# Sinica-SLAM/speechbrain

Hardware: AMD Instinct MI355X
Metric: audio-sec/sec Fbank→Conformer fwd (16kHz, B=32×15s) at 1/2/4/8 GPU (higher is better)
Workload: dtype bf16; 1 GPU; Fbank(80)→ConvFrontEnd(64,32)→Conformer 12L d=256 H=4 ffn=1024 k=31 encode, B=32×15s per GPU; global_batch=32, seq_len=376, parallelism=replicas1, hip_graph=True

## Files before the change

### speechbrain_amd/csrc/ffn.hip

```cpp
#include "mfma.h"

using namespace sbk;

namespace {

enum Act { ACT_NONE = 0, ACT_SWISH = 1, ACT_GLU = 2, ACT_LRELU = 3, ACT_GELU = 4 };

struct FfnArgs {
  const float* x;
  int M, H;
  const float *g0, *b0;
  float eps0;
  const bf16_t* img;
  const float* b1;
  int act;
  float slope;
  const float* b2;
  float alpha;
  const float *gp, *bp;
  float epsp;
  float* out;
  const float *gn, *bn;
  float epsn;
  void* u;
  int u_bf16;
  int np;
  bf16_t* yp;
  const float *g0b, *b0b;
  float eps0b;
  const float *b1b, *b2b;
  float alphab;
  float inv_n, npad;
  const bf16_t *sa, *simg;
  const float* sbias;
  int Kin, Tm;
  const float* rel_len;
  uint8_t* kpm_out;
};

__device__ __forceinline__ bf16x8 ld8(const bf16_t* p) { return *reinterpret_cast<const bf16x8*>(p); }

template <int V>
struct IntC {
  static constexpr int value = V;
};

constexpr int FFN_BM = 48;
#ifndef FFN_XCD_ORDER
#define FFN_XCD_ORDER 1
#endif
constexpr int FFN_PAD = 16;
constexpr int FFN_NW = 8, FFN_NT = FFN_NW * 64;
__device__ __forceinline__ constexpr int ffn_sw(int row) { return ((row >> 2) & 1) << 3; }
static_assert(FFN_NW % 8 == 0, "rows w + FFN_NW * i share bit 2 with w (their swizzle is ffn_sw(w))");
constexpr int FFN_RS = 12;

typedef float v2f __attribute__((ext_vector_type(2)));

#define FFN_MFMA(A, B, C) __builtin_amdgcn_mfma_f32_16x16x32_bf16((A), (B), (C), 0, 0, 0)

template <int ACT>
__device__ __forceinline__ float act_fn(float v, float slope) {
  if (ACT == ACT_SWISH) return v * __builtin_amdgcn_rcpf(1.0f + __expf(-v));
  if (ACT == ACT_LRELU) return v >= 0.f ? v : v * slope;
  if (ACT == ACT_GELU) return 0.5f * v * (1.0f + erff(v * 0.70710678118654752f));
  return v;
}

__device__ __forceinline__ f32x4 lds_f4(const float* p) {
  f32x4 v;
  const uint32_t la = (uint32_t)(uintptr_t)((const __attribute__((address_space(3))) float*)p);
  asm volatile("ds_read_b128 %0, %1" : "=v"(v) : "v"(la) : "memory");
  return v;
}

__device__ __forceinline__ uint32_t lds_addr(const void* p) {
  return (uint32_t)(uintptr_t)((const __attribute__((address_space(3))) char*)p);
}
__device__ __forceinline__ float lds_f1(const float* p) {
  float v;
  asm volatile("ds_read_b32 %0, %1" : "=v"(v) : "v"(lds_addr(p)) : "memory");
  return v;
}
__device__ __forceinline__ void lds_st1(float* p, float v) {
  asm volatile("ds_write_b32 %0, %1" ::"v"(lds_addr(p)), "v"(v) : "memory");
}
__device__ __forceinline__ void lds_st4(float* p, f32x4 v) {
  asm volatile("ds_write_b128 %0, %1" ::"v"(lds_addr(p)), "v"(v) : "memory");
}
__device__ __forceinline__ void lds_st2(void* p, uint2 v) {
  const unsigned long long u = (unsigned long long)v.x | ((unsigned long long)v.y << 32);
  asm volatile("ds_write_b64 %0, %1" ::"v"(lds_addr(p)), "v"(u) : "memory");
}
template <typename V>
__device__ __forceinline__ void tie(V& v) {
  asm volatile("s_waitcnt lgkmcnt(0)" : "+v"(v));
}
__device__ __forceinline__ void lds_barrier() {
  asm volatile("s_waitcnt lgkmcnt(0)" ::: "memory");
  __builtin_amdgcn_s_barrier();
}

__device__ __forceinline__ f32x4 gld4(const float* p) {
  f32x4 v;
  asm volatile("global_load_dwordx4 %0, %1, off" : "=v"(v) : "v"(p) : "memory");
  return v;
}
__device__ __forceinline__ void vtie(f32x4& v) { asm volatile("" : "+v"(v)); }

__device__ __forceinline__ void vm_wait(int n) {
  switch (n) {
    case 0: asm volatile("s_waitcnt vmcnt(0)" ::: "memory"); break;
    case 1: asm volatile("s_waitcnt vmcnt(1)" ::: "memory"); break;
    case 2: asm volatile("s_waitcnt vmcnt(2)" ::: "memory"); break;
    case 3: asm volatile("s_waitcnt vmcnt(3)" ::: "memory"); break;
    case 4: asm volatile("s_waitcnt vmcnt(4)" ::: "memory"); break;
    case 5: asm volatile("s_waitcnt vmcnt(5)" ::: "memory"); break;
    case 6: asm volatile("s_waitcnt vmcnt(6)" ::: "memory"); break;
    case 7: asm volatile("s_waitcnt vmcnt(7)" ::: "memory"); break;
    default: asm volatile("s_waitcnt vmcnt(8)" ::: "memory"); break;
  }
}

template <int D, int T2, int MT, int NW>
__device__ __forceinline__ void row_ln(float (&z)[T2][MT][4], float* red, const float* gam, const float* bet, float eps,
                                       int w, int g, int fr, float inv_n, float npad) {
  static_assert(NW == 8, "two b128 reads per row");
  float mean[MT], rstd[MT];
#pragma unroll
  for (int pass = 0; pass < 2; ++pass) {
    float part[MT];
#pragma unroll
    for (int mt = 0; mt < MT; ++mt) {
      float s = 0.f;
#pragma unroll
      for (int j = 0; j < T2; ++j)
#pragma unroll
        for (int e = 0; e < 4; ++e) {
          const float dv = pass ? z[j][mt][e] - mean[mt] : z[j][mt][e];
          s += pass ? dv * dv : dv;
        }
      part[mt] = col4_sum(s);
    }
    lds_barrier();
    if (g == 0) {
#pragma unroll
      for (int mt = 0; mt < MT; ++mt) lds_st1(red + (mt * 16 + fr) * FFN_RS + w, part[mt]);
    }
    lds_barrier();
    f32x4 rv[MT][2];
#pragma unroll
    for (int mt = 0; mt < MT; ++mt) {
      rv[mt][0] = lds_f4(red + (mt * 16 + fr) * FFN_RS);
      rv[mt][1] = lds_f4(red + (mt * 16 + fr) * FFN_RS + 4);
    }
#pragma unroll
    for (int mt = 0; mt < MT; ++mt) {
      tie(rv[mt][0]);
      tie(rv[mt][1]);
      const float t = (rv[mt][0][0] + rv[mt][0][1]) + (rv[mt][0][2] + rv[mt][0][3]) + (rv[mt][1][0] + rv[mt][1][1]) +
                      (rv[mt][1][2] + rv[mt][1][3]);
      if (pass)
        rstd[mt] = __builtin_amdgcn_rsqf((t - npad * mean[mt] * mean[mt]) * inv_n + eps);
      else
        mean[mt] = t * inv_n;
    }
  }
  f32x4 gv[T2], bv[T2];
#pragma unroll
  for (int j = 0; j < T2; ++j) {
    const int d = (w * T2 + j) * 16 + 4 * g;
    gv[j] = lds_f4(gam + d);
    bv[j] = lds_f4(bet + d);
  }
#pragma unroll
  for (int j = 0; j < T2; ++j) {
    tie(gv[j]);
    tie(bv[j]);
#pragma unroll
    for (int e = 0; e < 4; e += 2)
#pragma unroll
      for (int mt = 0; mt < MT; ++mt) {
        const v2f y = (v2f{z[j][mt][e], z[j][mt][e + 1]} - v2f{mean[mt], mean[mt]}) * v2f{rstd[mt], rstd[mt]} *
                          v2f{gv[j][e], gv[j][e + 1]} + v2f{bv[j][e], bv[j][e + 1]};
        z[j][mt][e] = y[0];
        z[j][mt][e + 1] = y[1];
      }
  }
}

__device__ __forceinline__ uint4 proj_pair(const f32x4& v0, const f32x4& v1) {
  const uint32_t a0 = pack_bf16x2(v0[0], v0[1]), a1 = pack_bf16x2(v0[2], v0[3]);
  const uint32_t b0 = pack_bf16x2(v1[0], v1[1]), b1 = pack_bf16x2(v1[2], v1[3]);
  const auto lo = __builtin_amdgcn_permlane16_swap(a0, b0, false, false);
  const auto hi = __builtin_amdgcn_permlane16_swap(a1, b1, false, false);
  return make_uint4(lo[0], hi[0], lo[1], hi[1]);
}

template <int K1, int KS, int MT, int XS, int BK>
__device__ __forceinline__ void load_frags(bf16x8 (&xa)[K1][KS][MT], const bf16_t* Xn, int fr, int fk) {
#pragma unroll
  for (int r = 0; r < K1; ++r)
#pragma unroll
    for (int ks = 0; ks < KS; ++ks)
#pragma unroll
      for (int mt = 0; mt < MT; ++mt)
        asm volatile("ds_read_b128 %0, %1"
                     : "=v"(xa[r][ks][mt])
                     : "v"(lds_addr(Xn + (mt * 16 + fr) * XS + r * BK + ks * 32 + fk))
                     : "memory");
#pragma unroll
  for (int r = 0; r < K1; ++r)
#pragma unroll
    for (int ks = 0; ks < KS; ++ks)
#pragma unroll
      for (int mt = 0; mt < MT; ++mt) tie(xa[r][ks][mt]);
}

SBK_PROBE_BUFFER(g_ffn_tl, 16, 256)
#define FFN_TL(i) SBK_PROBE(if (tl_rec >= 0 && lane == 0) g_ffn_tl[tl_rec][i] = __builtin_amdgcn_s_memtime();)

#include "convstage.h"

template <int D, int ACT, bool PROJ, bool CHAIN, bool CONV, bool SRC = false>
__device__ __forceinline__ void ffn_body(const FfnArgs& a, const ConvStageArgs* cs) {
  static_assert(!(CONV && SRC), "one kind of prologue");
  constexpr int BM = FFN_BM, HC = 256, NW = FFN_NW, NT = FFN_NT;
  constexpr int XS = D + FFN_PAD, HS = HC + FFN_PAD;
  constexpr int MT = BM / 16;
  constexpr int T = 256 / 16 / FFN_NW;
  constexpr int BK = 64;
  constexpr int K1 = D / BK, K2 = HC / BK, SPC = K1 + K2;
  constexpr int NB = 2;
  constexpr int TROWS = 256;
  constexpr int GL = TROWS * BK * 2 / 16 / NT;
  static_assert(GL * 8 == T * 16, "each wave stages exactly the weight rows it multiplies");
  constexpr int PER = D / 64;
  static_assert(PER == 4 && D == 256 && HC / 16 / NW == T && D / 16 / NW == T, "shape");

  extern __shared__ __attribute__((aligned(16))) unsigned char smem[];
  bf16_t* ring = reinterpret_cast<bf16_t*>(smem);
  bf16_t* Xn = ring + NB * TROWS * BK;
  bf16_t* Hs = Xn + BM * XS;
  float* b1s = reinterpret_cast<float*>(Hs + 2 * BM * HS);
  float* red = b1s + (CHAIN ? 2 : 1) * a.H;
  float* prm = red + BM * FFN_RS;
  enum { P_B2 = 0, P_GP, P_BP, P_G0B, P_B0B, P_B2B, P_GN, P_BN, P_N };
  static_assert(P_N == NW, "one parameter row per wave");

  const int tid = threadIdx.x, lane = tid & 63, w = tid >> 6;
  const int fr = lane & 15, g = lane >> 4, fk = (8 * g) ^ ffn_sw(fr);
  const int tile = CONV && FFN_XCD_ORDER ? xcd_tile(gridDim.x, blockIdx.x) : (int)blockIdx.x;
  int m0 = tile * BM, mlim = a.M;
  if constexpr (CONV) {
    const int nblk = (cs->T + BM - 1) / BM, b = tile / nblk;
    m0 = b * cs->T + (tile - b * nblk) * BM;
    mlim = (b + 1) * cs->T;
  }
  const int NCH = a.H / HC;
  const int S = NCH * SPC;
  const int SF = CHAIN ? 2 * S : S;
  const int SP = PROJ ? (a.np / TROWS) * K1 : 0;
  const int ST = SF + SP;
  SBK_PROBE(const int tl_rec = blockIdx.x == 128 ? w : blockIdx.x == 127 ? NW + w : -1;)
  FFN_TL(0);

  auto issue = [&](int s, int slot) __attribute__((always_inline)) {
    const bf16_t* src = a.img + (long long)s * (TROWS * BK) + w * (GL * 512) + lane * 8;
    bf16_t* dst = ring + slot * (TROWS * BK) + w * (GL * 512);
    const auto gs = (const __attribute__((address_space(1))) void*)src;
    const auto ls = (__attribute__((address_space(3))) void*)dst;
    static_assert(GL == 4, "four 1-KB pieces per wave and tile");
    __builtin_amdgcn_global_load_lds(gs, ls, 16, 0, 0);
    __builtin_amdgcn_global_load_lds(gs, ls, 16, 1024, 0);
    __builtin_amdgcn_global_load_lds(gs, ls, 16, 2048, 0);
    __builtin_amdgcn_global_load_lds(gs, ls, 16, 3072, 0);
  };
  constexpr int NRW = (BM + NW - 1) / NW;
  f32x4 xres[T][MT];
  if constexpr (CONV || SRC) {
    static_assert(T == 2 && MT == CS_MT3, "conv_stage hands over the chain's residual layout");
    constexpr int HS_END = (NB * TROWS * BK + BM * XS + 2 * BM * HS) * 2;
    float* ga0 = reinterpret_cast<float*>(smem + (CONV ? CS_LDS : HS_END - 2 * D * 4));
    static_assert(CS_LDS + 2 * D * 4 <= HS_END, "LN0 affine below b1");
    static_assert(CS_LDS >= (NB * TROWS * BK + BM * XS + BM * HS) * 2, "LN0 affine in the second hidden buffer");
    const float* psrc = w == P_B2 ? a.b2 : w == P_GP ? a.gp : w == P_BP ? a.bp : w == P_G0B ? a.g0b
                      : w == P_B0B ? a.b0b : w == P_B2B ? a.b2b : w == P_GN ? a.gn : a.bn;
    const bool b1t = tid * 4 < a.H;
    const float4 z4 = make_float4(0.f, 0.f, 0.f, 0.f);
    float4 pv = z4, b1v = z4, b1bv = z4, gav = z4;
    if (psrc) pv = *reinterpret_cast<const float4*>(psrc + lane * PER);
    if (b1t) {
      b1v = *reinterpret_cast<const float4*>(a.b1 + tid * 4);
      if (CHAIN) b1bv = *reinterpret_cast<const float4*>(a.b1b + tid * 4);
    }
    if (tid < D / 2) gav = *reinterpret_cast<const float4*>((tid < D / 4 ? a.g0 : a.b0) + 4 * (tid % (D / 4)));
    auto stage_params = [&]() __attribute__((always_inline)) {
      if (psrc) *reinterpret_cast<float4*>(prm + w * D + lane * PER) = pv;
      if (b1t) {
        *reinterpret_cast<float4*>(b1s + tid * 4) = b1v;
        if (CHAIN) *reinterpret_cast<float4*>(b1s + a.H + tid * 4) = b1bv;
      }
      if (tid < D / 2) *reinterpret_cast<float4*>(ga0 + 4 * tid) = gav;
    };
    if constexpr (CONV) {
      const int nblk = (cs->T + BM - 1) / BM, ub = tile / nblk;
      conv_stage(*cs, a.inv_n, a.npad, smem, ub, (tile - ub * nblk) * BM, xres, stage_params);
    } else {
      bf16_t* As = Xn;
      const int AS = a.Kin + FFN_PAD, KS = a.Kin / BK, cpr = a.Kin / 8;
      constexpr int NRA = BM / NW;
      static_assert(NRA * NW == BM && 768 / 8 <= 2 * 64, "two chunks per lane cover a row");
      bf16x8 av[NRA * 2];
#pragma unroll
      for (int i = 0; i < NRA * 2; ++i) {
        const int ch = min(lane + 64 * (i & 1), cpr - 1);
        av[i] = ld8(a.sa + (long long)min(m0 + w + NW * (i >> 1), mlim - 1) * a.Kin + ch * 8);
      }
      f32x4 sb[T];
#pragma unroll
      for (int j = 0; j < T; ++j) {
        sb[j] = f32x4{0.f, 0.f, 0.f, 0.f};
        if (a.sbias) sb[j] = *reinterpret_cast<const f32x4*>(a.sbias + (w * T + j) * 16 + 4 * g);
      }
      if (a.rel_len && tid < BM && m0 + tid < mlim) {
        const int m = m0 + tid, ub = m / a.Tm;
        a.kpm_out[m] = length_mask_byte(a.rel_len[ub], m - ub * a.Tm, a.Tm);
      }
#pragma unroll
      for (int i = 0; i < NRA * 2; ++i) {
        const int ch = lane + 64 * (i & 1);
        if (ch < cpr) *reinterpret_cast<bf16x8*>(As + (w + NW * (i >> 1)) * AS + ch * 8) = av[i];
      }
      stage_params();
      __syncthreads();
      auto issue_src = [&](int s, int slot) __attribute__((always_inline)) {
        const bf16_t* src = a.simg + (long long)s * (TROWS * BK) + w * (GL * 512) + lane * 8;
        bf16_t* dst = ring + slot * (TROWS * BK) + w * (GL * 512);
        const auto gs = (const __attribute__((address_space(1))) void*)src;
        const auto ls = (__attribute__((address_space(3))) void*)dst;
        __builtin_amdgcn_global_load_lds(gs, ls, 16, 0, 0);
        __builtin_amdgcn_global_load_lds(gs, ls, 16, 1024, 0);
        __builtin_amdgcn_global_load_lds(gs, ls, 16, 2048, 0);
        __builtin_amdgcn_global_load_lds(gs, ls, 16, 3072, 0);
      };
      issue_src(0, 0);
      issue_src(min(1, KS - 1), 1);
      f32x4 accs[T][MT];
#pragma unroll
      for (int t = 0; t < T; ++t)
#pragma unroll
        for (int mt = 0; mt < MT; ++mt) accs[t][mt] = f32x4{0.f, 0.f, 0.f, 0.f};
      for (int s = 0; s < KS; ++s) {
        asm volatile("s_waitcnt vmcnt(%0)" ::"n"(GL * (NB - 1)) : "memory");
        const bf16_t* tile = ring + (s % NB) * TROWS * BK;
        bf16x8 fw[BK / 32][T], fa[BK / 32][MT];
#pragma unroll
        for (int ks = 0; ks < BK / 32; ++ks) {
#pragma unroll
          for (int t = 0; t < T; ++t) {
            const int row = w * (T * 16) + t * 16 + fr;
            fw[ks][t] = ld8(tile + row * BK + (((ks * 4 + g) ^ ((row >> 1) & 7)) << 3));
          }
#pragma unroll
          for (int mt = 0; mt < MT; ++mt) fa[ks][mt] = ld8(As + (mt * 16 + fr) * AS + s * BK + ks * 32 + 8 * g);
        }
        asm volatile("s_waitcnt lgkmcnt(0)" ::: "memory");
        issue_src(min(s + NB, KS - 1), s % NB);
#pragma unroll
        for (int ks = 0; ks < BK / 32; ++ks)
#pragma unroll
          for (int t = 0; t < T; ++t)
#pragma unroll
            for (int mt = 0; mt < MT; ++mt) accs[t][mt] = FFN_MFMA(fw[ks][t], fa[ks][mt], accs[t][mt]);
      }
      asm volatile("s_waitcnt vmcnt(0)" ::: "memory");
#pragma unroll
      for (int j = 0; j < T; ++j)
#pragma unroll
        for (int mt = 0; mt < MT; ++mt) xres[j][mt] = accs[j][mt] + sb[j];
    }
    lds_barrier();
    issue(0, 0);
    issue(1, 1);
    float z[T][MT][4];
#pragma unroll
    for (int j = 0; j < T; ++j)
#pragma unroll
      for (int mt = 0; mt < MT; ++mt)
#pragma unroll
        for (int e = 0; e < 4; ++e) z[j][mt][e] = xres[j][mt][e];
    row_ln<D, T, MT, NW>(z, red, ga0, ga0 + D, a.eps0, w, g, fr, a.inv_n, a.npad);
#pragma unroll
    for (int j = 0; j < T; ++j) {
      const int d = (w * T + j) * 16 + 4 * g;
#pragma unroll
      for (int mt = 0; mt < MT; ++mt) {
        uint2 pk;
        pk.x = pack_bf16x2(z[j][mt][0], z[j][mt][1]);
        pk.y = pack_bf16x2(z[j][mt][2], z[j][mt][3]);
        lds_st2(Xn + (mt * 16 + fr) * XS + (d ^ ffn_sw(fr)), pk);
      }
    }
  } else {
#pragma unroll
  for (int j = 0; j < T; ++j)
#pragma unroll
    for (int mt = 0; mt < MT; ++mt) {
      const int row = min(m0 + mt * 16 + fr, mlim - 1);
      xres[j][mt] = gld4(a.x + (long long)row * D + (w * T + j) * 16 + 4 * g);
    }
  f32x4 xv[NRW];
#pragma unroll
  for (int i = 0; i < NRW; ++i) {
    const int rr = w + i * NW, row = min(m0 + rr, mlim - 1);
    xv[i] = gld4(a.x + (long long)row * D + lane * PER);
  }
  f32x4 g04 = gld4(a.g0 + lane * PER), b04 = gld4(a.b0 + lane * PER);
  const float* psrc = w == P_B2 ? a.b2 : w == P_GP ? a.gp : w == P_BP ? a.bp : w == P_G0B ? a.g0b
                    : w == P_B0B ? a.b0b : w == P_B2B ? a.b2b : w == P_GN ? a.gn : a.bn;
  f32x4 pv = f32x4{0.f, 0.f, 0.f, 0.f}, b1v = pv, b1bv = pv;
  if (psrc) pv = gld4(psrc + lane * PER);
  const bool b1t = tid * 4 < a.H;
  if (b1t) b1v = gld4(a.b1 + tid * 4);
  if (CHAIN && b1t) b1bv = gld4(a.b1b + tid * 4);
  issue(0, 0);
  issue(1, 1);
  asm volatile("s_waitcnt vmcnt(%0)" ::"n"(NB * GL) : "memory");
#pragma unroll
  for (int j = 0; j < T; ++j)
#pragma unroll
    for (int mt = 0; mt < MT; ++mt) vtie(xres[j][mt]);
#pragma unroll
  for (int i = 0; i < NRW; ++i) vtie(xv[i]);
  vtie(g04);
  vtie(b04);
  vtie(pv);
  vtie(b1v);
  vtie(b1bv);

#pragma unroll
  for (int i = 0; i < NRW; ++i) {
    const int rr = w + i * NW;
    if (rr >= BM) break;
    const bool live = m0 + rr < mlim;
    const float v[4] = {live ? xv[i][0] : 0.f, live ? xv[i][1] : 0.f, live ? xv[i][2] : 0.f, live ? xv[i][3] : 0.f};
    const float mean = wave_sum_v(v[0] + v[1] + v[2] + v[3]) * a.inv_n;
    float q = 0.f;
#pragma unroll
    for (int e = 0; e < 4; ++e) q += (v[e] - mean) * (v[e] - mean);
    const float rstd = __builtin_amdgcn_rsqf((wave_sum_v(q) - a.npad * mean * mean) * a.inv_n + a.eps0);
    uint2 pk;
    pk.x = pack_bf16x2((v[0] - mean) * rstd * g04[0] + b04[0], (v[1] - mean) * rstd * g04[1] + b04[1]);
    pk.y = pack_bf16x2((v[2] - mean) * rstd * g04[2] + b04[2], (v[3] - mean) * rstd * g04[3] + b04[3]);
    lds_st2(Xn + rr * XS + ((lane * PER) ^ ffn_sw(w)), pk);
  }
  static_assert(2048 <= NT * 4, "b1 in one float4 per thread");
  if (psrc) lds_st4(prm + w * D + lane * PER, pv);
  if (b1t) lds_st4(b1s + tid * 4, b1v);
  if (CHAIN && b1t) lds_st4(b1s + a.H + tid * 4, b1bv);
  }

  f32x4 acc1[T][MT], acc2[T][MT];
#pragma unroll
  for (int t = 0; t < T; ++t)
#pragma unroll
    for (int mt = 0; mt < MT; ++mt) {
      acc1[t][mt] = f32x4{0.f, 0.f, 0.f, 0.f};
      acc2[t][mt] = f32x4{0.f, 0.f, 0.f, 0.f};
    }

  FFN_TL(1);
  lds_barrier();
  bf16x8 xa[K1][BK / 32][MT];
  load_frags<K1, BK / 32, MT, XS, BK>(xa, Xn, fr, fk);
  auto step = [&](int s, int r, bool ph2, const bf16_t* Hc, bool bar, auto&& post) __attribute__((always_inline)) {
    asm volatile("s_waitcnt vmcnt(%0)" ::"n"(GL * (NB - 1)) : "memory");
    asm volatile("s_waitcnt lgkmcnt(0)" ::: "memory");
    if (bar) __builtin_amdgcn_s_barrier();
    if (s < 96) FFN_TL(2 + 2 * s);
    const bf16_t* tile = ring + (s % NB) * TROWS * BK;
    bf16x8 fw[BK / 32][T], fa[BK / 32][MT];
#pragma unroll
    for (int ks = 0; ks < BK / 32; ++ks) {
#pragma unroll
      for (int t = 0; t < T; ++t) {
        const int row = w * (T * 16) + t * 16 + fr;
        fw[ks][t] = ld8(tile + row * BK + (((ks * 4 + g) ^ ((row >> 1) & 7)) << 3));
      }
#pragma unroll
      for (int mt = 0; mt < MT; ++mt)
        fa[ks][mt] = ph2 ? ld8(Hc + (mt * 16 + fr) * HS + r * BK + ks * 32 + fk) : xa[ph2 ? 0 : r][ks][mt];
    }
    asm volatile("s_waitcnt lgkmcnt(0)" ::: "memory");
    issue(min(s + NB, ST - 1), s % NB);
#pragma unroll
    for (int ks = 0; ks < BK / 32; ++ks)
#pragma unroll
      for (int t = 0; t < T; ++t)
#pragma unroll
        for (int mt = 0; mt < MT; ++mt) {
          if (ph2)
            acc2[t][mt] = FFN_MFMA(fw[ks][t], fa[ks][mt], acc2[t][mt]);
          else
            acc1[t][mt] = FFN_MFMA(fw[ks][t], fa[ks][mt], acc1[t][mt]);
        }
    post();
    if (s < 96) FFN_TL(3 + 2 * s);
  };
  auto none = []() __attribute__((always_inline)) {};
  auto act_tiles = [&](int i0, int i1, const float* b1c, bf16_t* Hn) __attribute__((always_inline)) {
#pragma unroll
    for (int t = 0; t < T; ++t) {
      if ((t + 1) * MT <= i0 || t * MT >= i1) continue;
      const int n = w * (T * 16) + t * 16 + 4 * g;
      f32x4 bb;
      asm volatile("ds_read_b128 %0, %1\n\ts_waitcnt lgkmcnt(0)" : "=v"(bb) : "v"(lds_addr(b1c + n)) : "memory");
#pragma unroll
      for (int mt = 0; mt < MT; ++mt) {
        const int i = t * MT + mt;
        if (i < i0 || i >= i1) continue;
        const f32x4 v = acc1[t][mt];
        uint2 pk;
        pk.x = pack_bf16x2(act_fn<ACT>(v[0] + bb[0], a.slope), act_fn<ACT>(v[1] + bb[1], a.slope));
        pk.y = pack_bf16x2(act_fn<ACT>(v[2] + bb[2], a.slope), act_fn<ACT>(v[3] + bb[3], a.slope));
        const unsigned long long pv = (unsigned long long)pk.x | ((unsigned long long)pk.y << 32);
        asm volatile("ds_write_b64 %0, %1" ::"v"(lds_addr(Hn + (mt * 16 + fr) * HS + (n ^ ffn_sw(fr)))), "v"(pv) : "memory");
        acc1[t][mt] = f32x4{0.f, 0.f, 0.f, 0.f};
      }
    }
  };
  for (int stage = 0; stage < (CHAIN ? 2 : 1); ++stage) {
  if (CHAIN && stage == 1) {
    FFN_TL(197);
    float z[T][MT][4];
#pragma unroll
    for (int j = 0; j < T; ++j) {
      const int d = (w * T + j) * 16 + 4 * g;
      f32x4 bb = lds_f4(prm + P_B2 * D + d);
      tie(bb);
#pragma unroll
      for (int mt = 0; mt < MT; ++mt) {
        const f32x4 xr = xres[j][mt];
#pragma unroll
        for (int e = 0; e < 4; e += 2) {
          const v2f zz = v2f{xr[e], xr[e + 1]} +
                         v2f{a.alpha, a.alpha} * (v2f{acc2[j][mt][e], acc2[j][mt][e + 1]} + v2f{bb[e], bb[e + 1]});
          z[j][mt][e] = zz[0];
          z[j][mt][e + 1] = zz[1];
        }
        acc1[j][mt] = f32x4{0.f, 0.f, 0.f, 0.f};
        acc2[j][mt] = f32x4{0.f, 0.f, 0.f, 0.f};
      }
    }
    FFN_TL(200);
    if (a.gp) row_ln<D, T, MT, NW>(z, red, prm + P_GP * D, prm + P_BP * D, a.epsp, w, g, fr, a.inv_n, a.npad);
    FFN_TL(201);
#pragma unroll
    for (int j = 0; j < T; ++j)
#pragma unroll
      for (int mt = 0; mt < MT; ++mt) xres[j][mt] = f32x4{z[j][mt][0], z[j][mt][1], z[j][mt][2], z[j][mt][3]};
    row_ln<D, T, MT, NW>(z, red, prm + P_G0B * D, prm + P_B0B * D, a.eps0b, w, g, fr, a.inv_n, a.npad);
    FFN_TL(202);
#pragma unroll
    for (int j = 0; j < T; ++j) {
      const int d = (w * T + j) * 16 + 4 * g;
#pragma unroll
      for (int mt = 0; mt < MT; ++mt) {
        uint2 pk;
        pk.x = pack_bf16x2(z[j][mt][0], z[j][mt][1]);
        pk.y = pack_bf16x2(z[j][mt][2], z[j][mt][3]);
        lds_st2(Xn + (mt * 16 + fr) * XS + (d ^ ffn_sw(fr)), pk);
      }
    }
    lds_barrier();
    FFN_TL(203);
    load_frags<K1, BK / 32, MT, XS, BK>(xa, Xn, fr, fk);
    FFN_TL(198);
  }
  const float* b1st = b1s + stage * a.H;
  for (int c = 0; c < NCH; ++c) {
    const int s0 = stage * S + c * SPC;
#pragma unroll
    for (int r = 0; r < K1; ++r) step(s0 + r, r, false, nullptr, false, none);
    bf16_t* Hc = Hs + (c & 1) * BM * HS;
    act_tiles(0, T * MT, b1st + c * HC, Hc);
#pragma unroll
    for (int p = 0; p < K2; ++p) step(s0 + K1 + p, p, true, Hc, p == 0, none);
  }
  }
  if (!PROJ) asm volatile("s_waitcnt vmcnt(0)" ::: "memory");
  FFN_TL(194);

  const float* b2f = prm + (CHAIN ? P_B2B : P_B2) * D;
  const float alphaf = CHAIN ? a.alphab : a.alpha;
  const bool postln = !CHAIN && a.gp;
  float z[T][MT][4];
#pragma unroll
  for (int j = 0; j < T; ++j) {
    const int d = (w * T + j) * 16 + 4 * g;
    f32x4 bb = lds_f4(b2f + d);
    tie(bb);
#pragma unroll
    for (int mt = 0; mt < MT; ++mt) {
      const f32x4 xr = xres[j][mt];
#pragma unroll
      for (int e = 0; e < 4; e += 2) {
        const v2f zz = v2f{xr[e], xr[e + 1]} +
                       v2f{alphaf, alphaf} * (v2f{acc2[j][mt][e], acc2[j][mt][e + 1]} + v2f{bb[e], bb[e + 1]});
        z[j][mt][e] = zz[0];
        z[j][mt][e + 1] = zz[1];
      }
    }
  }
  FFN_TL(195);
  if (postln) row_ln<D, T, MT, NW>(z, red, prm + P_GP * D, prm + P_BP * D, a.epsp, w, g, fr, a.inv_n, a.npad);
  if (PROJ) {
    float* Zo = reinterpret_cast<float*>(Hs);
    constexpr int ZS = D + 4;
    static_assert(BM * ZS * 4 <= 2 * BM * HS * 2, "out rows fit over Hs");
#pragma unroll
    for (int j = 0; j < T; ++j)
#pragma unroll
      for (int mt = 0; mt < MT; ++mt) xres[j][mt] = f32x4{z[j][mt][0], z[j][mt][1], z[j][mt][2], z[j][mt][3]};
    row_ln<D, T, MT, NW>(z, red, prm + P_GN * D, prm + P_BN * D, a.epsn, w, g, fr, a.inv_n, a.npad);
    FFN_TL(204);
#pragma unroll
    for (int j = 0; j < T; ++j) {
      const int d = (w * T + j) * 16 + 4 * g;
#pragma unroll
      for (int mt = 0; mt < MT; ++mt) {
        lds_st4(Zo + (mt * 16 + fr) * ZS + d, xres[j][mt]);
        uint2 pk;
        pk.x = pack_bf16x2(z[j][mt][0], z[j][mt][1]);
        pk.y = pack_bf16x2(z[j][mt][2], z[j][mt][3]);
        lds_st2(Xn + (mt * 16 + fr) * XS + (d ^ ffn_sw(fr)), pk);
      }
    }
    lds_barrier();
    FFN_TL(205);
    static_assert(MT <= K1, "stores of a column block fit in its steps");
    static_assert(T == 2, "a lane's two tiles of a row pair up into one 16-B store");
    const int ncp = a.np / TROWS;
    const bool full = m0 + BM <= mlim;
    uint4 yq[MT];
    auto kst = [&](int c, int r) __attribute__((always_inline)) { return r < MT ? (c == 0 ? T : 1) : 0; };
    for (int nc = 0; nc < ncp; ++nc) {
#pragma unroll
      for (int r = 0; r < K1; ++r) {
        const int s = SF + nc * K1 + r;
        const int k1 = r >= 1 ? kst(nc, r - 1) : nc > 0 ? kst(nc - 1, K1 - 1) : 0;
        const int k2 = r >= 2 ? kst(nc, r - 2) : nc > 0 ? kst(nc - 1, K1 + r - 2) : 0;
        vm_wait((s + 1 < ST ? GL : 0) + (full ? k1 + k2 : 0));
        const bf16_t* tile = ring + (s % NB) * TROWS * BK;
        int ln;
        asm volatile("v_mbcnt_lo_u32_b32 %0, -1, 0\n\tv_mbcnt_hi_u32_b32 %0, -1, %0" : "=v"(ln));
        const int lfr = ln & 15, lg = ln >> 4;
        bf16x8 fw[BK / 32][T];
#pragma unroll
        for (int ks = 0; ks < BK / 32; ++ks)
#pragma unroll
          for (int t = 0; t < T; ++t) {
            const int row = w * (T * 16) + t * 16 + lfr;
            fw[ks][t] = ld8(tile + row * BK + (((ks * 4 + lg) ^ ((row >> 1) & 7)) << 3));
          }
        bf16x8 fx[BK / 32][MT];
#pragma unroll
        for (int ks = 0; ks < BK / 32; ++ks)
#pragma unroll
          for (int mt = 0; mt < MT; ++mt) {
            const uint32_t la = (uint32_t)(uintptr_t)((const __attribute__((address_space(3))) bf16_t*)(
                Xn + (mt * 16 + fr) * XS + r * BK + ks * 32 + fk));
            asm volatile("ds_read_b128 %0, %1" : "=v"(fx[ks][mt]) : "v"(la) : "memory");
          }
        f32x4 ov[T];
        if (r < MT && full && nc == 0) {
#pragma unroll
          for (int j = 0; j < T; ++j) ov[j] = lds_f4(Zo + (r * 16 + lfr) * ZS + (w * T + j) * 16 + 4 * lg);
        }
        asm volatile("s_waitcnt lgkmcnt(0)" ::: "memory");
        if (s + NB < ST) issue(s + NB, s % NB);
        asm volatile("" ::: "memory");
        if (r < MT && full) {
          const long long row = m0 + r * 16 + lfr;
          if (nc == 0) {
#pragma unroll
            for (int j = 0; j < T; ++j)
              *reinterpret_cast<f32x4*>(a.out + row * D + (w * T + j) * 16 + 4 * lg) = ov[j];
          } else {
            *reinterpret_cast<uint4*>(a.yp + row * a.np + (nc - 1) * TROWS + w * (T * 16) + 16 * (lg & 1) + 8 * (lg >> 1)) =
                yq[r < MT ? r : 0];
          }
        }
#pragma unroll
        for (int ks = 0; ks < BK / 32; ++ks)
#pragma unroll
          for (int t = 0; t < T; ++t)
#pragma unroll
            for (int mt = 0; mt < MT; ++mt)
              acc1[t][mt] = __builtin_amdgcn_mfma_f32_16x16x32_bf16(fw[ks][t], fx[ks][mt], acc1[t][mt], 0, 0, 0);
      }
      int ln;
      asm volatile("v_mbcnt_lo_u32_b32 %0, -1, 0\n\tv_mbcnt_hi_u32_b32 %0, -1, %0" : "=v"(ln));
#pragma unroll
      for (int mt = 0; mt < MT; ++mt) {
        yq[mt] = proj_pair(acc1[0][mt], acc1[1][mt]);
        acc1[0][mt] = f32x4{0.f, 0.f, 0.f, 0.f};
        acc1[1][mt] = f32x4{0.f, 0.f, 0.f, 0.f};
        const int row = m0 + mt * 16 + (ln & 15), lg = ln >> 4;
        if ((!full || nc == ncp - 1) && row < mlim)
          *reinterpret_cast<uint4*>(a.yp + (long long)row * a.np + nc * TROWS + w * (T * 16) + 16 * (lg & 1) + 8 * (lg >> 1)) =
              yq[mt];
      }
    }
    FFN_TL(206);
    if (!full) {
      f32x4 ov[T][MT];
#pragma unroll
      for (int j = 0; j < T; ++j)
#pragma unroll
        for (int mt = 0; mt < MT; ++mt) ov[j][mt] = lds_f4(Zo + (mt * 16 + fr) * ZS + (w * T + j) * 16 + 4 * g);
      asm volatile("s_waitcnt lgkmcnt(0)" ::: "memory");
#pragma unroll
      for (int j = 0; j < T; ++j)
#pragma unroll
        for (int mt = 0; mt < MT; ++mt) {
          const int row = m0 + mt * 16 + fr;
          if (row < mlim) *reinterpret_cast<f32x4*>(a.out + (long long)row * D + (w * T + j) * 16 + 4 * g) = ov[j][mt];
        }
    }
    SBK_PROBE(asm volatile("s_waitcnt vmcnt(0)" ::: "memory");)
    FFN_TL(196);
    return;
  }
#pragma unroll
  for (int j = 0; j < T; ++j) {
    if (!a.out) break;
    const int d = (w * T + j) * 16 + 4 * g;
#pragma unroll
    for (int mt = 0; mt < MT; ++mt) {
      const int row = m0 + mt * 16 + fr;
      if (row < mlim)
        *reinterpret_cast<float4*>(a.out + (long long)row * D + d) =
            make_float4(z[j][mt][0], z[j][mt][1], z[j][mt][2], z[j][mt][3]);
    }
  }
  if (a.gn) {
    row_ln<D, T, MT, NW>(z, red, prm + P_GN * D, prm + P_BN * D, a.epsn, w, g, fr, a.inv_n, a.npad);
#pragma unroll
    for (int j = 0; j < T; ++j) {
      const int d = (w * T + j) * 16 + 4 * g;
#pragma unroll
      for (int mt = 0; mt < MT; ++mt) {
        const int row = m0 + mt * 16 + fr;
        if (row >= mlim) continue;
        if (a.u_bf16) {
          uint2 pk;
          pk.x = pack_bf16x2(z[j][mt][0], z[j][mt][1]);
          pk.y = pack_bf16x2(z[j][mt][2], z[j][mt][3]);
          *reinterpret_cast<uint2*>(reinterpret_cast<bf16_t*>(a.u) + (long long)row * D + d) = pk;
        } else {
          *reinterpret_cast<float4*>(reinterpret_cast<float*>(a.u) + (long long)row * D + d) =
              make_float4(z[j][mt][0], z[j][mt][1], z[j][mt][2], z[j][mt][3]);
        }
      }
    }
  }
  FFN_TL(196);
}

template <int D, int ACT, bool PROJ, bool CHAIN>
__global__ void __launch_bounds__(FFN_NT) ffn_kernel(FfnArgs a) {
  ffn_body<D, ACT, PROJ, CHAIN, false>(a, nullptr);
}

template <int ACT>
__global__ void __launch_bounds__(FFN_NT) conv_chain_kernel(FfnArgs a, ConvStageArgs c) {
  ffn_body<256, ACT, true, true, true>(a, &c);
}

template <int ACT>
__global__ void __launch_bounds__(FFN_NT) conv_tail_kernel(FfnArgs a, ConvStageArgs c) {
  ffn_body<256, ACT, false, false, true>(a, &c);
}

template <int ACT>
__global__ void __launch_bounds__(FFN_NT) src_ffn_kernel(FfnArgs a) {
  ffn_body<256, ACT, true, false, false, true>(a, nullptr);
}

template <int D>
size_t ffn_lds(int H, bool chain) {
  return ((size_t)2 * 256 * 64 + (size_t)FFN_BM * (D + FFN_PAD) + (size_t)2 * FFN_BM * (256 + FFN_PAD)) *
             sizeof(bf16_t) +
         (size_t)(chain ? 2 : 1) * H * 4 + (size_t)FFN_RS * FFN_BM * 4 + (size_t)FFN_NW * D * 4;
}

template <int D, int ACT, bool PROJ, bool CHAIN>
int launch_ffn_act(const FfnArgs& a, size_t lds, hipStream_t s) {
  if (hipError_t e = sbk::lds_optin(reinterpret_cast<const void*>(&ffn_kernel<D, ACT, PROJ, CHAIN>), lds))
    return (int)e;
  hipLaunchKernelGGL((ffn_kernel<D, ACT, PROJ, CHAIN>), dim3((a.M + FFN_BM - 1) / FFN_BM), dim3(FFN_NT), lds, s, a);
  return 0;
}

template <int D, bool PROJ, bool CHAIN>
int launch_ffn(const FfnArgs& a, hipStream_t s) {
  const size_t lds = ffn_lds<D>(a.H, CHAIN);
  if (lds > 160 * 1024) return SBK_ERR_ARG;
  switch (a.act) {
    case ACT_SWISH: return launch_ffn_act<D, ACT_SWISH, PROJ, CHAIN>(a, lds, s);
    case ACT_LRELU: return launch_ffn_act<D, ACT_LRELU, PROJ, CHAIN>(a, lds, s);
    case ACT_GELU: return launch_ffn_act<D, ACT_GELU, PROJ, CHAIN>(a, lds, s);
    case ACT_NONE: return launch_ffn_act<D, ACT_NONE, PROJ, CHAIN>(a, lds, s);
    default: return SBK_ERR_ARG;
  }
}

int ffn_dispatch(const FfnArgs& a, hipStream_t s) {
  const bool proj = a.np > 0, chain = a.g0b != nullptr;
  if (chain) return proj ? launch_ffn<256, true, true>(a, s) : launch_ffn<256, false, true>(a, s);
  return proj ? launch_ffn<256, true, false>(a, s) : launch_ffn<256, false, false>(a, s);
}

template <int ACT>
int launch_src_ffn_act(const FfnArgs& a, size_t lds, hipStream_t s) {
  if (hipError_t e = sbk::lds_optin(reinterpret_cast<const void*>(&src_ffn_kernel<ACT>), lds)) return (int)e;
  hipLaunchKernelGGL((src_ffn_kernel<ACT>), dim3((a.M + FFN_BM - 1) / FFN_BM), dim3(FFN_NT), lds, s, a);
  return 0;
}

int src_ffn_dispatch(const FfnArgs& a, hipStream_t s) {
  const size_t lds = ffn_lds<256>(a.H, false);
  if (lds > 160 * 1024 || (size_t)FFN_BM * (a.Kin + FFN_PAD) > (size_t)3 * FFN_BM * (256 + FFN_PAD) - 2 * 256 * 2)
    return SBK_ERR_ARG;
  switch (a.act) {
    case ACT_SWISH: return launch_src_ffn_act<ACT_SWISH>(a, lds, s);
    case ACT_LRELU: return launch_src_ffn_act<ACT_LRELU>(a, lds, s);
    case ACT_GELU: return launch_src_ffn_act<ACT_GELU>(a, lds, s);
    case ACT_NONE: return launch_src_ffn_act<ACT_NONE>(a, lds, s);
    default: return SBK_ERR_ARG;
  }
}

template <int ACT, bool TAIL>
int launch_conv_chain_act(const FfnArgs& a, const ConvStageArgs& c, unsigned grid, size_t lds, hipStream_t s) {
  const auto kern = TAIL ? &conv_tail_kernel<ACT> : &conv_chain_kernel<ACT>;
  if (hipError_t e = sbk::lds_optin(reinterpret_cast<const void*>(kern), lds)) return (int)e;
  hipLaunchKernelGGL(kern, dim3(grid), dim3(FFN_NT), lds, s, a, c);
  return 0;
}

template <bool TAIL>
int conv_chain_dispatch(const FfnArgs& a, const ConvStageArgs& c, hipStream_t s) {
  const size_t lds = ffn_lds<256>(a.H, !TAIL);
  static_assert(CS_LDS + 2 * 256 * 4 <= (2 * 256 * 64 + FFN_BM * (256 + FFN_PAD) * 3) * 2, "the conv stage lies under ring, Xn, Hs");
  if (lds > 160 * 1024) return SBK_ERR_ARG;
  const long long grid = (long long)c.B * ((c.T + FFN_BM - 1) / FFN_BM);
  if (grid > 0x7fffffffLL) return SBK_ERR_ARG;
  switch (a.act) {
    case ACT_SWISH: return launch_conv_chain_act<ACT_SWISH, TAIL>(a, c, (unsigned)grid, lds, s);
    case ACT_LRELU: return launch_conv_chain_act<ACT_LRELU, TAIL>(a, c, (unsigned)grid, lds, s);
    case ACT_GELU: return launch_conv_chain_act<ACT_GELU, TAIL>(a, c, (unsigned)grid, lds, s);
    case ACT_NONE: return launch_conv_chain_act<ACT_NONE, TAIL>(a, c, (unsigned)grid, lds, s);
    default: return SBK_ERR_ARG;
  }
}

__global__ void __launch_bounds__(256) conv_image_kernel(const bf16_t* __restrict__ w1p, const bf16_t* __restrict__ w2,
                                                         bf16_t* __restrict__ img) {
  const int n = (CS_P1T + CS_P3T) * 256 * 8;
  for (int i = blockIdx.x * blockDim.x + threadIdx.x; i < n; i += gridDim.x * blockDim.x) {
    const int s = i >> 11, rem = i & 2047, r = rem >> 3, jp = rem & 7;
    const int j = jp ^ ((r >> 1) & 7);
    const bf16_t* src = s < CS_P1T ? w1p + (long long)((r >> 5) * 64 + (s & 1) * 32 + (r & 31)) * CS_D + (s >> 1) * 64
                                   : w2 + (long long)r * CS_D + (s - CS_P1T) * 64;
    *reinterpret_cast<uint4*>(img + (long long)i * 8) = *reinterpret_cast<const uint4*>(src + 8 * j);
  }
}

__global__ void __launch_bounds__(256) wo_image_kernel(const bf16_t* __restrict__ wo, bf16_t* __restrict__ img) {
  const int n = CS_WOT * 256 * 8;
  for (int i = blockIdx.x * blockDim.x + threadIdx.x; i < n; i += gridDim.x * blockDim.x) {
    const int s = i >> 11, rem = i & 2047, r = rem >> 3, jp = rem & 7;
    const int j = jp ^ ((r >> 1) & 7);
    *reinterpret_cast<uint4*>(img + (long long)i * 8) =
        *reinterpret_cast<const uint4*>(wo + (long long)r * CS_D + s * 64 + 8 * j);
  }
}

__global__ void __launch_bounds__(CS_D) dw_image_kernel(const float* __restrict__ wc, const float* __restrict__ bc,
                                                        int K, uint32_t* __restrict__ img) {
  const int j = blockIdx.x, c = threadIdx.x;
  if (j == CS_NP) {
    img[j * CS_D + c] = __float_as_uint(bc ? bc[c] : 0.f);
    return;
  }
  const float lo = 2 * j < K ? wc[2 * j * CS_D + c] : 0.f;
  const float hi = 2 * j + 1 < K ? wc[(2 * j + 1) * CS_D + c] : 0.f;
  img[j * CS_D + c] = pack_bf16x2(lo, hi);
}

struct ImgSrc {
  const bf16_t *w1, *w2, *w1b, *w2b, *wp;
  int D, H, ntile_blk, ntile_ffn, chain;
};

__device__ __forceinline__ void img_tile_src(const ImgSrc& q, int s, const bf16_t** mat, int* ld, int* row0,
                                             int* k0) {
  const int K1 = q.D / 64, SPC = K1 + 4;
  if (s >= q.ntile_ffn) {
    const int pj = s - q.ntile_ffn, nc = pj / K1, r = pj - nc * K1;
    *mat = q.wp; *ld = q.D; *row0 = nc * 256; *k0 = r * 64;
    return;
  }
  const bool sb = s >= q.ntile_blk;
  const int sl = sb ? s - q.ntile_blk : s, c = sl / SPC, r = sl - c * SPC;
  if (r < K1) {
    *mat = sb ? q.w1b : q.w1; *ld = q.D; *row0 = c * 256; *k0 = r * 64;
  } else {
    *mat = sb ? q.w2b : q.w2; *ld = q.H; *row0 = 0; *k0 = c * 256 + (r - K1) * 64;
  }
}

__global__ void __launch_bounds__(256) ffn_image_kernel(ImgSrc q, int ntile, bf16_t* __restrict__ img) {
  const long long n = (long long)ntile * 256 * 8;
  for (long long i = (long long)blockIdx.x * blockDim.x + threadIdx.x; i < n; i += (long long)gridDim.x * blockDim.x) {
    const int s = (int)(i >> 11), rem = (int)(i & 2047), r = rem >> 3, jp = rem & 7;
    const bf16_t* mat;
    int ld, row0, k0;
    img_tile_src(q, s, &mat, &ld, &row0, &k0);
    const int j = jp ^ ((r >> 1) & 7);
    *reinterpret_cast<uint4*>(img + i * 8) =
        *reinterpret_cast<const uint4*>(mat + (long long)(row0 + r) * ld + k0 + 8 * j);
  }
}

int ffn_tiles(int D, int H, int np, int chain) {
  const int per_blk = (H / 256) * (D / 64 + 4);
  return (chain ? 2 : 1) * per_blk + (np / 256) * (D / 64);
}

}

SBK_PROBE_EXPORT(sbk_probe_ffn_tl, g_ffn_tl)

SBK_API int sbk_ffn_supported(int D, int H) { return D == 256 && H > 0 && H % 256 == 0 && H <= 2048; }

SBK_API long long sbk_ffn_image_elems(int D, int H, int np, int chain) {
  if (!sbk_ffn_supported(D, H) || np < 0 || np % 256) return -1;
  return (long long)ffn_tiles(D, H, np, chain) * 256 * 64;
}

SBK_API int sbk_ffn_image(const void* w1, const void* w2, const void* w1b, const void* w2b, const void* wp, int D,
                          int H, int np, void* img, void* stream) {
  const int chain = w1b != nullptr;
  if (!sbk_ffn_supported(D, H) || !w1 || !w2 || !img || (chain && !w2b) || np < 0 || np % 256 || (np > 0) != (wp != nullptr))
    return SBK_ERR_ARG;
  if ((reinterpret_cast<uintptr_t>(w1) | reinterpret_cast<uintptr_t>(w2) | reinterpret_cast<uintptr_t>(w1b) |
       reinterpret_cast<uintptr_t>(w2b) | reinterpret_cast<uintptr_t>(wp) | reinterpret_cast<uintptr_t>(img)) & 15)
    return SBK_ERR_ARG;
  ImgSrc q;
  q.w1 = reinterpret_cast<const bf16_t*>(w1); q.w2 = reinterpret_cast<const bf16_t*>(w2);
  q.w1b = reinterpret_cast<const bf16_t*>(w1b); q.w2b = reinterpret_cast<const bf16_t*>(w2b);
  q.wp = reinterpret_cast<const bf16_t*>(wp);
  q.D = D; q.H = H; q.chain = chain;
  q.ntile_blk = (H / 256) * (D / 64 + 4);
  q.ntile_ffn = (chain ? 2 : 1) * q.ntile_blk;
  const int nt = ffn_tiles(D, H, np, chain);
  const long long chunks = (long long)nt * 2048;
  hipLaunchKernelGGL(ffn_image_kernel, dim3((unsigned)std::min<long long>((chunks + 255) / 256, 4096)), dim3(256), 0,
                     (hipStream_t)stream, q, nt, reinterpret_cast<bf16_t*>(img));
  SBK_CHECK_LAUNCH();
  return 0;
}

namespace {
int ffn_check(const float* x, int M, int D, int H, const float* g0, const float* b0, const void* img,
              long long img_elems, int chain, const float* b1, int act, const float* b2, const float* gp,
              const float* bp, float* out, const float* gn, const float* bn, void* u, int np, void* yp,
              bool out_opt = false) {
  if (M <= 0 || !sbk_ffn_supported(D, H) || !g0 || !b0 || !img || !b1 || !b2 || (!out && !out_opt)) return SBK_ERR_ARG;
  if (np < 0 || np % 256 || img_elems != sbk_ffn_image_elems(D, H, np, chain)) return SBK_ERR_ARG;
  if (act == ACT_GLU || act < 0 || act > ACT_GELU || (gn && !u && np == 0)) return SBK_ERR_ARG;
// ... 260 lines not shown
```

Measured before the change: 439,300 audio-sec/sec.

## Reorder FFN up-projection k-steps by row half to overlap activation with MFMA

The first-GEMM weight tiles are now loaded per row half instead of per k step. The k=4 steps are regrouped so that the first output-row half (t=0) finishes after two steps. The activation of that half is then written to LDS while the second half's MFMAs run, either as a separate act_tiles call or interleaved per MFMA under FFN_ACT_VPM. This aims to hide the activation and LDS-write latency that sat between the two GEMM phases. In exchange, issue indexing and fragment addressing become more complex, and static_asserts now fix the shapes.

```diff
diff --git a/speechbrain_amd/csrc/ffn.hip b/speechbrain_amd/csrc/ffn.hip
--- a/speechbrain_amd/csrc/ffn.hip
+++ b/speechbrain_amd/csrc/ffn.hip
@@ -49,6 +49,12 @@
 #ifndef FFN_XCD_ORDER
 #define FFN_XCD_ORDER 1
 #endif
+#ifndef FFN_ACT_VPM
+#define FFN_ACT_VPM 0
+#endif
+#ifndef FFN_ACT_SPLIT
+#define FFN_ACT_SPLIT(ACT) ((ACT) == ACT_SWISH || (ACT) == ACT_GELU ? 2 : 1)
+#endif
 constexpr int FFN_PAD = 16;
 constexpr int FFN_NW = 8, FFN_NT = FFN_NW * 64;
 __device__ __forceinline__ constexpr int ffn_sw(int row) { return ((row >> 2) & 1) << 3; }
@@ -265,16 +271,28 @@
   SBK_PROBE(const int tl_rec = blockIdx.x == 128 ? w : blockIdx.x == 127 ? NW + w : -1;)
   FFN_TL(0);
 
-  auto issue = [&](int s, int slot) __attribute__((always_inline)) {
-    const bf16_t* src = a.img + (long long)s * (TROWS * BK) + w * (GL * 512) + lane * 8;
+  auto issue = [&](int s, int q, int slot) __attribute__((always_inline)) {
     bf16_t* dst = ring + slot * (TROWS * BK) + w * (GL * 512);
-    const auto gs = (const __attribute__((address_space(1))) void*)src;
     const auto ls = (__attribute__((address_space(3))) void*)dst;
     static_assert(GL == 4, "four 1-KB pieces per wave and tile");
-    __builtin_amdgcn_global_load_lds(gs, ls, 16, 0, 0);
-    __builtin_amdgcn_global_load_lds(gs, ls, 16, 1024, 0);
-    __builtin_amdgcn_global_load_lds(gs, ls, 16, 2048, 0);
-    __builtin_amdgcn_global_load_lds(gs, ls, 16, 3072, 0);
+    if (q < 0) {
+      const bf16_t* src = a.img + (long long)s * (TROWS * BK) + w * (GL * 512) + lane * 8;
+      const auto gs = (const __attribute__((address_space(1))) void*)src;
+      __builtin_amdgcn_global_load_lds(gs, ls, 16, 0, 0);
+      __builtin_amdgcn_global_load_lds(gs, ls, 16, 1024, 0);
+      __builtin_amdgcn_global_load_lds(gs, ls, 16, 2048, 0);
+      __builtin_amdgcn_global_load_lds(gs, ls, 16, 3072, 0);
+    } else {
+      const bf16_t* src =
+          a.img + (long long)(s - q + 2 * (q & 1)) * (TROWS * BK) + w * (GL * 512) + (q >> 1) * (GL * 256) + lane * 8;
+      const auto gs = (const __attribute__((address_space(1))) void*)src;
+      const auto gs2 = (const __attribute__((address_space(1))) void*)(src + TROWS * BK);
+      const auto ls2 = (__attribute__((address_space(3))) void*)(dst + GL * 256);
+      __builtin_amdgcn_global_load_lds(gs, ls, 16, 0, 0);
+      __builtin_amdgcn_global_load_lds(gs, ls, 16, 1024, 0);
+      __builtin_amdgcn_global_load_lds(gs2, ls2, 16, 0, 0);
+      __builtin_amdgcn_global_load_lds(gs2, ls2, 16, 1024, 0);
+    }
   };
   constexpr int NRW = (BM + NW - 1) / NW;
   f32x4 xres[T][MT];
@@ -381,8 +399,8 @@
         for (int mt = 0; mt < MT; ++mt) xres[j][mt] = accs[j][mt] + sb[j];
     }
     lds_barrier();
-    issue(0, 0);
-    issue(1, 1);
+    issue(0, 0, 0);
+    issue(1, 1, 1);
     float z[T][MT][4];
 #pragma unroll
     for (int j = 0; j < T; ++j)
@@ -424,8 +442,8 @@
   const bool b1t = tid * 4 < a.H;
   if (b1t) b1v = gld4(a.b1 + tid * 4);
   if (CHAIN && b1t) b1bv = gld4(a.b1b + tid * 4);
-  issue(0, 0);
-  issue(1, 1);
+  issue(0, 0, 0);
+  issue(1, 1, 1);
   asm volatile("s_waitcnt vmcnt(%0)" ::"n"(NB * GL) : "memory");
 #pragma unroll
   for (int j = 0; j < T; ++j)
@@ -474,41 +492,58 @@
   lds_barrier();
   bf16x8 xa[K1][BK / 32][MT];
   load_frags<K1, BK / 32, MT, XS, BK>(xa, Xn, fr, fk);
-  auto step = [&](int s, int r, bool ph2, const bf16_t* Hc, bool bar, auto&& post) __attribute__((always_inline)) {
+  static_assert(K1 == 4 && K2 == 4 && T == 2 && BK == 64, "two row halves by two k halves per chunk");
+  auto step = [&](int s, auto pc, const bf16_t* Hc, auto&& post, auto vpm) __attribute__((always_inline)) {
+    constexpr int P = decltype(pc)::value, VPM = decltype(vpm)::value;
+    constexpr bool ph2 = P >= K1;
     asm volatile("s_waitcnt vmcnt(%0)" ::"n"(GL * (NB - 1)) : "memory");
     asm volatile("s_waitcnt lgkmcnt(0)" ::: "memory");
-    if (bar) __builtin_amdgcn_s_barrier();
+    if (P == K1) __builtin_amdgcn_s_barrier();
     if (s < 96) FFN_TL(2 + 2 * s);
     const bf16_t* tile = ring + (s % NB) * TROWS * BK;
-    bf16x8 fw[BK / 32][T], fa[BK / 32][MT];
-#pragma unroll
-    for (int ks = 0; ks < BK / 32; ++ks) {
-#pragma unroll
-      for (int t = 0; t < T; ++t) {
-        const int row = w * (T * 16) + t * 16 + fr;
-        fw[ks][t] = ld8(tile + row * BK + (((ks * 4 + g) ^ ((row >> 1) & 7)) << 3));
-      }
-#pragma unroll
-      for (int mt = 0; mt < MT; ++mt)
-        fa[ks][mt] = ph2 ? ld8(Hc + (mt * 16 + fr) * HS + r * BK + ks * 32 + fk) : xa[ph2 ? 0 : r][ks][mt];
+    bf16x8 fw[T * (BK / 32)], fa[BK / 32][MT];
+#pragma unroll
+    for (int i = 0; i < T; ++i)
+#pragma unroll
+      for (int ks = 0; ks < BK / 32; ++ks)
+        fw[i * 2 + ks] = ld8(tile + w * (GL * 512) + i * (GL * 256) + fr * BK + (((ks * 4 + g) ^ ((fr >> 1) & 7)) << 3));
+    if constexpr (ph2) {
+#pragma unroll
+      for (int ks = 0; ks < BK / 32; ++ks)
+#pragma unroll
+        for (int mt = 0; mt < MT; ++mt) fa[ks][mt] = ld8(Hc + (mt * 16 + fr) * HS + (P - K1) * BK + ks * 32 + fk);
     }
     asm volatile("s_waitcnt lgkmcnt(0)" ::: "memory");
-    issue(min(s + NB, ST - 1), s % NB);
-#pragma unroll
-    for (int ks = 0; ks < BK / 32; ++ks)
-#pragma unroll
-      for (int t = 0; t < T; ++t)
-#pragma unroll
-        for (int mt = 0; mt < MT; ++mt) {
-          if (ph2)
-            acc2[t][mt] = FFN_MFMA(fw[ks][t], fa[ks][mt], acc2[t][mt]);
-          else
-            acc1[t][mt] = FFN_MFMA(fw[ks][t], fa[ks][mt], acc1[t][mt]);
+    if constexpr (P + NB < SPC) {
+      issue(s + NB, P + NB < K1 ? P + NB : -1, s % NB);
+    } else {
+      if (s + NB < SF)
+        issue(s + NB, P + NB - SPC, s % NB);
+      else
+        issue(min(s + NB, ST - 1), -1, s % NB);
+    }
+    if constexpr (VPM > 0) __builtin_amdgcn_sched_barrier(0);
+    if constexpr (ph2) {
+#pragma unroll
+      for (int ks = 0; ks < BK / 32; ++ks)
+#pragma unroll
+        for (int t = 0; t < T; ++t)
+#pragma unroll
+          for (int mt = 0; mt < MT; ++mt) acc2[t][mt] = FFN_MFMA(fw[t * 2 + ks], fa[ks][mt], acc2[t][mt]);
+    } else {
+#pragma unroll
+      for (int j = 0; j < 2 * (BK / 32); ++j)
+#pragma unroll
+        for (int mt = 0; mt < MT; ++mt)
+        {
+          acc1[P >> 1][mt] = FFN_MFMA(fw[j], xa[(P & 1) * 2 + (j >> 1)][j & 1][mt], acc1[P >> 1][mt]);
+          if constexpr (VPM > 0) post(j * MT + mt);
         }
-    post();
+    }
+    if constexpr (VPM == 0) post(-1);
     if (s < 96) FFN_TL(3 + 2 * s);
   };
-  auto none = []() __attribute__((always_inline)) {};
+  auto none = [](int) __attribute__((always_inline)) {};
   auto act_tiles = [&](int i0, int i1, const float* b1c, bf16_t* Hn) __attribute__((always_inline)) {
 #pragma unroll
     for (int t = 0; t < T; ++t) {
@@ -581,12 +616,34 @@
   const float* b1st = b1s + stage * a.H;
   for (int c = 0; c < NCH; ++c) {
     const int s0 = stage * S + c * SPC;
-#pragma unroll
-    for (int r = 0; r < K1; ++r) step(s0 + r, r, false, nullptr, false, none);
     bf16_t* Hc = Hs + (c & 1) * BM * HS;
-    act_tiles(0, T * MT, b1st + c * HC, Hc);
-#pragma unroll
-    for (int p = 0; p < K2; ++p) step(s0 + K1 + p, p, true, Hc, p == 0, none);
+    const float* b1c = b1st + c * HC;
+    step(s0, IntC<0>{}, nullptr, none, IntC<0>{});
+    step(s0 + 1, IntC<1>{}, nullptr, none, IntC<0>{});
+    f32x4 bbu;
+    float ru[4];
+    auto under = [&](int i, int mt0, int mt1) __attribute__((always_inline)) {
+      if (i < 0) return act_tiles(mt0, mt1, b1c, Hc);
+      const int n = w * (T * 16) + 4 * g;
+      if (i == 0) asm volatile("ds_read_b128 %0, %1\n\ts_waitcnt lgkmcnt(0)" : "=v"(bbu) : "v"(lds_addr(b1c + n)) : "memory");
+      const int mt = mt0 + (i >> 2), e = i & 3;
+      if (mt < mt1) {
+        ru[e] = act_fn<ACT>(acc1[0][mt][e] + bbu[e], a.slope);
+        if (e == 3) {
+          const unsigned long long pv = (unsigned long long)pack_bf16x2(ru[0], ru[1]) | ((unsigned long long)pack_bf16x2(ru[2], ru[3]) << 32);
+          asm volatile("ds_write_b64 %0, %1" ::"v"(lds_addr(Hc + (mt * 16 + fr) * HS + (n ^ ffn_sw(fr)))), "v"(pv) : "memory");
+          acc1[0][mt] = f32x4{0.f, 0.f, 0.f, 0.f};
+        }
+      }
+      __builtin_amdgcn_sched_barrier(0);
+    };
+    step(s0 + 2, IntC<2>{}, nullptr, [&](int i) __attribute__((always_inline)) { under(i, 0, FFN_ACT_SPLIT(ACT)); }, IntC<FFN_ACT_VPM>{});
+    step(s0 + 3, IntC<3>{}, nullptr, [&](int i) __attribute__((always_inline)) { under(i, FFN_ACT_SPLIT(ACT), MT); }, IntC<FFN_ACT_VPM>{});
+    act_tiles(MT, T * MT, b1c, Hc);
+    step(s0 + 4, IntC<4>{}, Hc, none, IntC<0>{});
+    step(s0 + 5, IntC<5>{}, Hc, none, IntC<0>{});
+    step(s0 + 6, IntC<6>{}, Hc, none, IntC<0>{});
+    step(s0 + 7, IntC<7>{}, Hc, none, IntC<0>{});
   }
   }
   if (!PROJ) asm volatile("s_waitcnt vmcnt(0)" ::: "memory");
@@ -679,7 +736,7 @@
           for (int j = 0; j < T; ++j) ov[j] = lds_f4(Zo + (r * 16 + lfr) * ZS + (w * T + j) * 16 + 4 * lg);
         }
         asm volatile("s_waitcnt lgkmcnt(0)" ::: "memory");
-        if (s + NB < ST) issue(s + NB, s % NB);
+        if (s + NB < ST) issue(s + NB, -1, s % NB);
         asm volatile("" ::: "memory");
         if (r < MT && full) {
           const long long row = m0 + r * 16 + lfr;
```

Result: slower. 433,600 audio-sec/sec (-1.3%).
